# apschera2023uzk/MWR_fast_forward_operators_and_LBLs

Hardware: AMD Instinct MI355X
Metric: TB evaluations/sec (profile x channel x angle) (higher is better)
Workload: dtype f64

## Files before the change

### mwr_fast_forward_operators_and_lbls_amd/csrc/mwrt_absorption.hip.h

```cpp
#pragma once
#include "mwrt_math.hip.h"

namespace mwrt {

typedef const __attribute__((address_space(4))) LineMasks* cmasks;
__device__ __forceinline__ LineMasks load_masks(const LineMasks* table, int chunk) {
  const cmasks q = (cmasks)table + chunk;
  LineMasks lm;
  lm.o2_far = q->o2_far; lm.h2o_far = q->h2o_far; lm.h2o_none = q->h2o_none; lm.h2o_res = q->h2o_res; lm.h2o_sd = q->h2o_sd;
  lm.h2o_sdfar = q->h2o_sdfar; lm.h2o_sdint = q->h2o_sdint;
  lm.h2o_vfar = q->h2o_vfar; lm.o2_vfar = q->o2_vfar; lm.vf_u0 = q->vf_u0; lm.vf_h = q->vf_h; lm.vf_invh = q->vf_invh;
  return lm;
}

struct LevelState {
  double t;
  double p;
  double rho;
  double pdry;
};

__device__ __forceinline__ double goff_gratch_e(double tk, double rh) {
  const double LN10 = 2.302585092994045684;
  const double INV_LN10 = 0.434294481903251828;
  double y = 373.16 / tk;
  double es = -7.90298 * (y - 1.0) + 5.02808 * (flog(y) * INV_LN10)
            - 1.3816e-07 * (fexp(LN10 * (11.344 * (1.0 - (1.0 / y)))) - 1.0)
            + 0.0081328 * (fexp(LN10 * (-3.49149 * (y - 1.0))) - 1.0) + 3.0057148979490314 ;
  return rh * fexp(LN10 * es);
}

__device__ __forceinline__ LevelState level_state(double p_hpa, double tk, double e) {
  const double rvap = (0.01 * 8.314510) / 18.01528;
  double v = 300.0 / tk;
  double ekpa = e / 10.0;
  double pdrykpa = p_hpa / 10.0 - ekpa;
  LevelState s;
  s.t = 300.0 / v;
  s.p = (pdrykpa + ekpa) * 10.0;
  s.rho = ekpa * 10.0 / (rvap * s.t);
  s.pdry = pdrykpa * 10.0;
  return s;
}

struct H2OLine {
  double c1;
  double w0, wsq;
  double sw;
  double sbase;
  double s;
  double base;
};

__device__ __forceinline__ H2OLine h2o_line(cmodel M, int k, double pda, double pvap, double ti, double tiln,
                                            double ti2, bool shifted) {
  H2OLine q;
  const auto& R = M->h2or[k];
  const double fl = R.fl;
  q.w0 = R.w0 * pda * fexp(R.x * tiln) + R.w0s * pvap * fexp(R.xs * tiln);
  double shift = 0.0;
  if (shifted) {
    const double xh = R.xh, xhs = R.xhs, aa = R.aair, as = R.aself;
    double sf = R.sh * pda, ss = R.shs * pvap;
    if (aa != 0.0) sf *= (1.0 - aa * tiln);
    if (as != 0.0) ss *= (1.0 - as * tiln);
    if (xh != 0.0) sf *= fexp(xh * tiln);
    if (xhs != 0.0) ss *= fexp(xhs * tiln);
    shift = sf + ss;
  }
  q.wsq = q.w0 * q.w0;
  q.s = R.s1 * ti2 * fexp(R.b2 * (1.0 - ti));
  q.base = fdiv1(q.w0, 562500.0 + q.wsq);
  q.c1 = fl + shift;
  q.sw = q.s * q.w0;
  q.sbase = q.s * q.base;
  return q;
}

struct FarLine { double P, Q, A2, Bc; };

template <int NFC>
__device__ __forceinline__ void far_quad_accumulate(const double* sfq, const FarLine& a, const FarLine& b,
                                                    const FarLine& c, const FarLine& d, double (&sum)[NFC]) {
  static_assert(NFC % 2 == 0, "frequencies are taken in pairs");
  auto front = [&](const double (&f2s)[2], double (&den)[2], double (&num)[2]) {
#pragma unroll
    for (int g = 0; g < 2; ++g) {
      const double f2 = f2s[g];
      const double d0 = __builtin_fma(f2, f2 + a.A2, a.Bc);
      const double d1 = __builtin_fma(f2, f2 + b.A2, b.Bc);
      const double d2 = __builtin_fma(f2, f2 + c.A2, c.Bc);
      const double d3 = __builtin_fma(f2, f2 + d.A2, d.Bc);
      const double n0 = __builtin_fma(f2, a.P, a.Q);
      const double n1 = __builtin_fma(f2, b.P, b.Q);
      const double n2 = __builtin_fma(f2, c.P, c.Q);
      const double n3 = __builtin_fma(f2, d.P, d.Q);
      const double p01 = d0 * d1, p23 = d2 * d3;
      const double m01 = __builtin_fma(n0, d1, n1 * d0);
      const double m23 = __builtin_fma(n2, d3, n3 * d2);
      den[g] = p01 * p23;
      num[g] = __builtin_fma(m01, p23, m23 * p01);
    }
  };
  double den[2], num[2], r[2];
  double f2c[2] = {sfq[1], sfq[3]};
  double f2n[2] = {sfq[(NFC > 2) ? 5 : 1], sfq[(NFC > 2) ? 7 : 3]};
  front(f2c, den, num);
  r[0] = __builtin_amdgcn_rcp(den[0]); r[1] = __builtin_amdgcn_rcp(den[1]);
#pragma unroll
  for (int j = 0; j < NFC; j += 2) {
    double den_n[2] = {1.0, 1.0}, num_n[2] = {0.0, 0.0}, f2p[2] = {0.0, 0.0};
    if (j + 4 < NFC) { f2p[0] = sfq[2 * (j + 4) + 1]; f2p[1] = sfq[2 * (j + 5) + 1]; }
    MWRT_STAGE();
    if (j + 2 < NFC) front(f2n, den_n, num_n);
    MWRT_STAGE();
    const double e0 = __builtin_fma(-den[0], r[0], 1.0), e1 = __builtin_fma(-den[1], r[1], 1.0);
    r[0] = __builtin_fma(r[0], e0, r[0]); r[1] = __builtin_fma(r[1], e1, r[1]);
    sum[j] = __builtin_fma(num[0], r[0], sum[j]); sum[j + 1] = __builtin_fma(num[1], r[1], sum[j + 1]);
    if (j + 2 < NFC) {
      den[0] = den_n[0]; den[1] = den_n[1]; num[0] = num_n[0]; num[1] = num_n[1];
      r[0] = __builtin_amdgcn_rcp(den[0]); r[1] = __builtin_amdgcn_rcp(den[1]);
      f2n[0] = f2p[0]; f2n[1] = f2p[1];
    }
  }
  MWRT_STAGE();
}

constexpr int VF_TERMS = 8;
__device__ __forceinline__ void vfar_add(const FarLine& fl, double u0, double h, double (&acc)[VF_TERMS]) {
  const double d0 = __builtin_fma(u0, u0 + fl.A2, fl.Bc);
  const double d1h = __builtin_fma(fl.A2, h, (2.0 * u0) * h);
  double rd = __builtin_amdgcn_rcp(d0);
  rd = __builtin_fma(rd, __builtin_fma(-d0, rd, 1.0), rd);
  const double a = -d1h * rd, b = (-(h * h)) * rd;
  double cm2 = __builtin_fma(fl.P, u0, fl.Q) * rd;
  double cm1 = __builtin_fma(a, cm2, (fl.P * h) * rd);
  acc[0] += cm2;
  acc[1] += cm1;
#pragma unroll
  for (int j = 2; j < VF_TERMS; ++j) {
    const double cj = __builtin_fma(a, cm1, b * cm2);
    acc[j] += cj;
    cm2 = cm1; cm1 = cj;
  }
}
template <int NFC>
__device__ __forceinline__ void vfar_eval(const double* sfq, double invh, double mu , const double (&acc)[VF_TERMS], double (&sum)[NFC]) {
  constexpr int G = (NFC % 7 == 0) ? 7 : ((NFC % 4 == 0) ? 4 : 2);
  static_assert(NFC % G == 0, "group width");
#pragma unroll
  for (int j0 = 0; j0 < NFC; j0 += G) {
    double x[G], p[G];
#pragma unroll
    for (int g = 0; g < G; ++g) { x[g] = __builtin_fma(sfq[2 * (j0 + g) + 1], invh, mu); p[g] = acc[VF_TERMS - 1]; }
#pragma unroll
    for (int k = VF_TERMS - 2; k >= 0; --k) {
#pragma unroll
      for (int g = 0; g < G; ++g) p[g] = __builtin_fma(p[g], x[g], acc[k]);
      MWRT_STAGE();
    }
#pragma unroll
    for (int g = 0; g < G; ++g) sum[j0 + g] += p[g];
  }
}

template <int NFC>
__device__ __forceinline__ void far_pair_accumulate(const double* sfq, const FarLine& a, const FarLine& b, double (&sum)[NFC]) {
#pragma unroll
  for (int j = 0; j < NFC; ++j) {
    const double f2 = sfq[2 * j + 1];
    const double d0 = __builtin_fma(f2, f2 + a.A2, a.Bc);
    const double d1 = __builtin_fma(f2, f2 + b.A2, b.Bc);
    const double n0 = __builtin_fma(f2, a.P, a.Q);
    const double n1 = __builtin_fma(f2, b.P, b.Q);
    const double den = d0 * d1;
    const double num = __builtin_fma(n0, d1, n1 * d0);
    double r = __builtin_amdgcn_rcp(den);
    r = __builtin_fma(r, __builtin_fma(-den, r, 1.0), r);
    sum[j] = __builtin_fma(num, r, sum[j]);
  }
}

__device__ __forceinline__ unsigned long long lowest_bits(unsigned long long m, int n) {
  unsigned long long out = 0;
  for (int i = 0; i < n; ++i) { const unsigned long long b = m & (0ull - m); out |= b; m ^= b; }
  return out;
}


template <int NFC, bool NODES = false>
__device__ __forceinline__ void h2o_absorb(cmodel M, const LevelState& L, const double* sfq ,
                                           const LineMasks& lm, double (&awet)[NFC], unsigned excl = 0u,
                                           const double* init_sum = nullptr, double init_bsum = 0.0,
                                           unsigned* failed = nullptr, double* bsum_out = nullptr,
                                           cdoubles sdw = nullptr ) {
  const double t = L.t;
  const double pvap = fdiv(L.rho * t, M->h2o_pvap_div);
  const double pda = L.p - pvap;
  const double den = M->h2o_den_coef * L.rho;
  const double lnc = flog(fdiv(M->h2o_reftcon, t));
  const double con0 = (M->h2o_cf * pda * fexp(M->h2o_xcf * lnc) + M->h2o_cs * pvap * fexp(M->h2o_xcs * lnc)) * pvap;
  const double ti = fdiv(M->h2o_reftline, t);
  const double tiln = flog(ti);
  const double ti2 = fexp(2.5 * tiln);
  const bool shifted = M->h2o_shift_mode != 0;
  double sum[NFC];
#pragma unroll
  for (int j = 0; j < NFC; ++j) sum[j] = init_sum ? init_sum[j] : 0.0;

  const int nl = M->n_h2o;
  const unsigned all = ((nl >= 32) ? 0xffffffffu : ((1u << nl) - 1u)) & ~excl;
  const double fmin = sfq[2 * NFC], fmax = sfq[2 * NFC + 1];
  double bsum = init_bsum;
  const unsigned sd_eff = lm.h2o_sd & ~lm.h2o_sdfar;
  unsigned sd_extra = 0u;
  unsigned deferred = (~lm.h2o_far | lm.h2o_res) & ~sd_eff & ~lm.h2o_none & all;
  const unsigned setA = (MWRT_ABLATE & 2) ? 0u : (lm.h2o_far & ~lm.h2o_res & ~sd_eff & ~lm.h2o_none & all);
  const unsigned setV = NODES ? 0u : (setA & lm.h2o_vfar);
  const unsigned setQ = setA & ~setV;
  const unsigned leftA = (unsigned)lowest_bits(setQ, __builtin_popcount(setQ) & 3);
  const unsigned leftP = (__builtin_popcount(leftA) >= 2) ? (unsigned)lowest_bits(leftA, 2) : 0u;
  deferred |= leftA & ~leftP;
  auto far_setup = [&](int k, FarLine& fl) {
    const H2OLine q = h2o_line(M, k, pda, pvap, ti, tiln, ti2, shifted);
    const bool plain = wave_all_of(q.c1 - fmin < 750.0, fmax - q.c1 < 750.0, q.c1 - fmin > -750.0, fmax + q.c1 < 750.0, fmin + q.c1 > -750.0);
    const double cc = __builtin_fma(q.c1, q.c1, q.wsq);
    fl.A2 = 2.0 * __builtin_fma(-q.c1, q.c1, q.wsq);
    fl.Bc = cc * cc;
    double P = 2.0 * q.sw, bs = 2.0 * q.sbase;
    const bool sdline = M->h2o_w2[k] > 0.0;
    const bool reach = sdline && !wave_all(10.0 * q.w0 < ::fmin(fabs(q.c1 - fmin), fabs(q.c1 - fmax)));
    if (reach || !plain) {
      if constexpr (NODES) *failed |= 1u << k;
      else if (reach) sd_extra |= 1u << k;
      else deferred |= 1u << k;
      P = 0.0; bs = 0.0;
    }
    fl.P = P;
    fl.Q = P * cc;
    bsum += bs;
  };
  if (setV) {
    double acc[VF_TERMS];
#pragma unroll
    for (int j = 0; j < VF_TERMS; ++j) acc[j] = 0.0;
    for (unsigned m = setV; m; m &= m - 1u) {
      FarLine q;
      far_setup(__builtin_ctz(m), q);
      vfar_add(q, lm.vf_u0, lm.vf_h, acc);
    }
    LDS_RELOAD_FENCE();
    vfar_eval<NFC>(sfq, lm.vf_invh, -lm.vf_u0 * lm.vf_invh, acc, sum);
  }
  for (unsigned m = setQ & ~leftA; m;) {
    FarLine q0, q1, q2, q3;
    far_setup(__builtin_ctz(m), q0); m &= m - 1u;
    far_setup(__builtin_ctz(m), q1); m &= m - 1u;
    far_setup(__builtin_ctz(m), q2); m &= m - 1u;
    far_setup(__builtin_ctz(m), q3); m &= m - 1u;
    LDS_RELOAD_FENCE();
    far_quad_accumulate<NFC>(sfq, q0, q1, q2, q3, sum);
  }
  if (leftP) {
    FarLine q0, q1;
    unsigned m = leftP;
    far_setup(__builtin_ctz(m), q0); m &= m - 1u;
    far_setup(__builtin_ctz(m), q1);
    LDS_RELOAD_FENCE();
    far_pair_accumulate<NFC>(sfq, q0, q1, sum);
  }
  if (MWRT_ABLATE & 2) deferred = 0u;
  for (unsigned m = deferred; m; m &= m - 1u) {
    const int k = __builtin_ctz(m);
    const H2OLine q = h2o_line(M, k, pda, pvap, ti, tiln, ti2, shifted);
    const bool d1_in = (q.c1 - fmin < 750.0) && (fmax - q.c1 < 750.0) && (q.c1 - fmin > -750.0);
    const bool d1_out = (q.c1 - fmax >= 750.0) || (fmin - q.c1 >= 750.0);
    const bool d2_in = fmax + q.c1 < 750.0 && fmin + q.c1 > -750.0;
    const bool d2_out = fmin + q.c1 >= 750.0;
    if (wave_all(d1_out && d2_out)) continue;
    if (M->h2o_w2[k] > 0.0 && !wave_all(10.0 * q.w0 < ::fmin(fabs(q.c1 - fmin), fabs(q.c1 - fmax)))) {
      if constexpr (NODES) *failed |= 1u << k; else sd_extra |= 1u << k;
      continue;
    }
    LDS_RELOAD_FENCE();
    if (wave_all(d1_in && d2_in)) {
      bsum = __builtin_fma(2.0, q.sbase, bsum);
#pragma unroll
      for (int j = 0; j < NFC; ++j) {
        const double f = sfq[2 * j];
        const double d1 = f - q.c1;
        const double d2 = f + q.c1;
        const double D1 = __builtin_fma(d1, d1, q.wsq);
        const double D2 = __builtin_fma(d2, d2, q.wsq);
        const double den12 = D1 * D2;
        double r = __builtin_amdgcn_rcp(den12);
        r = __builtin_fma(r, __builtin_fma(-den12, r, 1.0), r);
        sum[j] = __builtin_fma((D1 + D2) * r, q.sw, sum[j]);
      }
    } else if (wave_all(d1_in && d2_out)) {
      bsum += q.sbase;
#pragma unroll
      for (int j = 0; j < NFC; ++j) {
        const double d1 = sfq[2 * j] - q.c1;
        const double D1 = __builtin_fma(d1, d1, q.wsq);
        double r = __builtin_amdgcn_rcp(D1);
        r = __builtin_fma(r, __builtin_fma(-D1, r, 1.0), r);
        sum[j] = __builtin_fma(r, q.sw, sum[j]);
      }
    } else if constexpr (NODES) {
      *failed |= 1u << k;
    } else {
#pragma unroll
      for (int j = 0; j < NFC; ++j) {
        const double f = sfq[2 * j];
        const double d1 = f - q.c1;
        const double d2 = f + q.c1;
        const double D1 = __builtin_fma(d1, d1, q.wsq);
        const double D2 = __builtin_fma(d2, d2, q.wsq);
        const double m1 = (fabs(d1) < 750.0) ? 1.0 : 0.0;
        const double m2 = (fabs(d2) < 750.0) ? 1.0 : 0.0;
        const double num = __builtin_fma(m2, D1, m1 * D2);
        const double r = fdiv1(num, D1 * D2);
        sum[j] = __builtin_fma(r, q.sw, sum[j]);
        sum[j] = __builtin_fma(-(m1 + m2), q.sbase, sum[j]);
      }
    }
  }
  if constexpr (NODES) {
#pragma unroll
    for (int j = 0; j < NFC; ++j) awet[j] = sum[j];
    *bsum_out = bsum;
    return;
  }
#pragma unroll
  for (int j = 0; j < NFC; ++j) sum[j] -= bsum;
  const unsigned setC = (MWRT_ABLATE & 4) ? 0u : ((sd_eff | sd_extra) & all);
  for (unsigned m = setC; m; m &= m - 1u) {
// ... 27 lines not shown
        sum[j] -= inner ? q.sbase : sbase2;
      }
    } else {
#pragma unroll
      for (int j = 0; j < NFC; ++j) {
        const double f = sfq[2 * j];
        const double d1 = f - q.c1;
        const double d2 = f + q.c1;
        const double D1 = __builtin_fma(d1, d1, q.wsq);
        const double D2 = __builtin_fma(d2, d2, q.wsq);
        const double a1 = fabs(d1);
        const double m1 = (a1 < 750.0 && !(a1 < sdlim)) ? 1.0 : 0.0;
        const double m2 = (fabs(d2) < 750.0) ? 1.0 : 0.0;
        const double num = __builtin_fma(m2, D1, m1 * D2);
        const double r = fdiv1(num, D1 * D2);
        sum[j] = __builtin_fma(r, q.sw, sum[j]);
        sum[j] = __builtin_fma(-(m1 + m2), q.sbase, sum[j]);
      }
    }
    LDS_RELOAD_FENCE();
    auto sd_shape = [&](double d1) -> double {
      const cplx xc = cmul(cplx{xre, d1 + xim0}, iden2);
      const cplx xrt = csqrt_principal(xc);
      const cplx w = dcerror_upper(-xrt.im, xrt.re);
      const cplx pxw = cmul(cplx{1.77245385090551603 * xrt.re, 1.77245385090551603 * xrt.im}, w);
      return __builtin_fma(2.0 * (1.0 - pxw.re), iden2.re, 2.0 * pxw.im * iden2.im);
    };
    bool done = false;
    if constexpr (NFC == 16 && !NODES) {
      if (half) {
        done = true;
        const double dmin = ::fmin(fabs(sfq[0] - q.c1), fabs(sfq[2 * 15] - q.c1));
        if (wave_any(dmin < sdlim)) {
          double dn[SD_NODES];
#pragma unroll
          for (int n = 0; n < SD_NODES; ++n) {
            const int j = sd_node_slot(n);
            const double d1 = sfq[2 * j] - q.c1;
            const double sdre = sd_shape(d1);
            const double lres = fdiv1(q.w0, __builtin_fma(d1, d1, q.wsq));
            dn[n] = sdre - lres;
            const double r1 = (fabs(d1) < sdlim) ? sdre - q.base : 0.0;
            sum[j] = __builtin_fma(q.s, r1, sum[j]);
          }
#pragma unroll
          for (int i = 0; i < SD_TARGETS; ++i) {
            const int j = 2 * i + 1;
            double dl = 0.0;
#pragma unroll
            for (int n = 0; n < SD_NODES; ++n) dl = __builtin_fma(sdw[i * SD_NODES + n], dn[n], dl);
            const bool inner = fabs(sfq[2 * j] - q.c1) < sdlim;
            sum[j] = __builtin_fma(q.s, inner ? dl : 0.0, sum[j]);
          }
        }
      }
    }
    if (!done) {
#pragma unroll
      for (int j = 0; j < NFC; ++j) {
        const double d1 = sfq[2 * j] - q.c1;
        const bool inner = fabs(d1) < sdlim;
        if (wave_any(inner)) {
          const double r1 = inner ? sd_shape(d1) - q.base : 0.0;
          sum[j] = __builtin_fma(q.s, r1, sum[j]);
        }
      }
    }
  }
  const bool dry = !(L.rho > 0.0);
#pragma unroll
  for (int j = 0; j < NFC; ++j) {
    const double f2 = sfq[2 * j + 1];
    awet[j] = dry ? 0.0 : (3.183e-05 * den * sum[j] + con0) * f2;
  }
}

struct O2Line {
  double c1, df2;
  double P, Q;
  double cc;
  double dnu;
};

template <int NFC, bool NODES = false>
__device__ __forceinline__ void dry_absorb(cmodel M, const LevelState& L, const double* sfq ,
                                           const LineMasks& lm, double (&adry)[NFC], unsigned long long excl = 0ull,
                                           const double* init_sum = nullptr, unsigned long long* failed = nullptr) {
  const double temp = L.t;
  const double pres = L.p;
  const double th = fdiv(300.0, temp);
  const double th1 = th - 1.0;
  const double lnth = flog(th);
  const double b = fexp(M->o2_x * lnth);
  const double preswv = fdiv(L.rho * temp, M->o2_pvap_div);
  const double presda = pres - preswv;
  const double den = 0.001 * (presda * b + M->o2_wv_factor * preswv * th);
  const double dens = 0.001 * (presda + M->o2_wv_factor * preswv) * th;
  const double dfnr = M->o2_wb300 * den;
  const double pe2 = den * den;
  const bool second = M->o2_mix_mode != 0;
  const double ymul = second ? den : 0.001 * pres * b;
  const bool line1_dens = !second && M->o2_line1_dens;

  double sum[NFC];
#pragma unroll
  for (int j = 0; j < NFC; ++j) sum[j] = init_sum ? init_sum[j] : 0.0;

  long long be_prev = -1;
  double ebe = 1.0;
  auto line_setup = [&](int k) -> O2Line {
    const auto& R = M->o2r[k];
    const double y = ymul * __builtin_fma(R.y1, th1, R.y0);
    double dnu = 0.0, gfac = 1.0;
    if (second) {
      dnu = pe2 * __builtin_fma(R.dnu1, th1, R.dnu0);
      gfac = __builtin_fma(pe2, __builtin_fma(R.g1, th1, R.g0), 1.0);
    }
    const double df = R.w300 * ((k == 0 && line1_dens) ? dens : den);
    const long long be_bits = __builtin_bit_cast(long long, R.be);
    if (be_bits != be_prev) { ebe = fexp(-R.be * th1); be_prev = be_bits; }
    const double str = R.s300rf2 * ebe;
    O2Line q;
    q.dnu = dnu;
    q.c1 = R.f + dnu;
    q.df2 = df * df;
    const double a = (str * df) * gfac;
    const double cb = q.c1 * (str * y);
    q.cc = __builtin_fma(q.c1, q.c1, q.df2);
    q.P = a + cb;
    q.Q = q.cc * (a - cb);
    return q;
  };

  const int nl = M->n_o2;
  const unsigned long long all = ((nl >= 64) ? ~0ull : ((1ull << nl) - 1ull)) & ~excl;
  unsigned long long near = ~lm.o2_far & all;
  const unsigned long long setA = (MWRT_ABLATE & 1) ? 0ull : (lm.o2_far & all);
  const unsigned long long setV = NODES ? 0ull : (setA & lm.o2_vfar);
  const unsigned long long setQ = setA & ~setV;
  const unsigned long long leftA = lowest_bits(setQ, __builtin_popcountll(setQ) & 3);
  const unsigned long long leftP = (__builtin_popcountll(leftA) >= 2) ? lowest_bits(leftA, 2) : 0ull;
  near |= leftA & ~leftP;
  auto far_setup = [&](int k, FarLine& fl) {
    const O2Line q = line_setup(k);
    double P = q.P, Q = q.Q;
    if (!NODES && second && !wave_all(fabs(q.dnu) < FAR_SHIFT_GHZ)) { near |= 1ull << k; P = 0.0; Q = 0.0; }
    fl.P = P; fl.Q = Q;
    fl.A2 = 2.0 * __builtin_fma(-q.c1, q.c1, q.df2);
    fl.Bc = q.cc * q.cc;
  };
  if (setV) {
    double acc[VF_TERMS];
#pragma unroll
    for (int j = 0; j < VF_TERMS; ++j) acc[j] = 0.0;
    for (unsigned long long m = setV; m; m &= m - 1ull) {
      FarLine q;
      far_setup(__builtin_ctzll(m), q);
      vfar_add(q, lm.vf_u0, lm.vf_h, acc);
    }
    LDS_RELOAD_FENCE();
    vfar_eval<NFC>(sfq, lm.vf_invh, -lm.vf_u0 * lm.vf_invh, acc, sum);
  }
  for (unsigned long long m = setQ & ~leftA; m;) {
    FarLine q0, q1, q2, q3;
    far_setup(__builtin_ctzll(m), q0); m &= m - 1ull;
    far_setup(__builtin_ctzll(m), q1); m &= m - 1ull;
    far_setup(__builtin_ctzll(m), q2); m &= m - 1ull;
    far_setup(__builtin_ctzll(m), q3); m &= m - 1ull;
    LDS_RELOAD_FENCE();
    far_quad_accumulate<NFC>(sfq, q0, q1, q2, q3, sum);
  }
  if (leftP) {
    FarLine q0, q1;
    unsigned long long m = leftP;
    far_setup(__builtin_ctzll(m), q0); m &= m - 1ull;
    far_setup(__builtin_ctzll(m), q1);
    LDS_RELOAD_FENCE();
    far_pair_accumulate<NFC>(sfq, q0, q1, sum);
  }
  if (MWRT_ABLATE & 1) near = 0ull;
  be_prev = -1;
  for (unsigned long long m = near; m; m &= m - 1ull) {
    const int k = __builtin_ctzll(m);
    const O2Line q = line_setup(k);
    LDS_RELOAD_FENCE();
#pragma unroll
    for (int j = 0; j < NFC; ++j) {
      const double f = sfq[2 * j], f2 = sfq[2 * j + 1];
      const double d1 = f - q.c1;
      const double d2 = f + q.c1;
      const double D1 = __builtin_fma(d1, d1, q.df2);
      const double D2 = __builtin_fma(d2, d2, q.df2);
      const double den12 = D1 * D2;
      double r = __builtin_amdgcn_rcp(den12);
      r = __builtin_fma(r, __builtin_fma(-den12, r, 1.0), r);
      sum[j] = __builtin_fma(__builtin_fma(f2, q.P, q.Q), r, sum[j]);
    }
  }
  if constexpr (NODES) {
#pragma unroll
    for (int j = 0; j < NFC; ++j) adry[j] = sum[j];
    (void)failed;
    return;
  }
  const double scale2 = 2.0 * M->o2_coef * presda * th * th * th;
  const double pn2 = M->n2_ptot ? pres : L.pdry;
  const double n2c = M->n2_n * M->n2_l * pn2 * pn2 * fexp(M->n2_m * lnth);
  const double nr0 = 0.5 * M->o2_nonres * dfnr;
  const double dfnr2 = dfnr * dfnr;
#pragma unroll
  for (int j = 0; j < NFC; ++j) {
    const double f2 = sfq[2 * j + 1];
    const double hnonres = fdiv(nr0 * f2, th * (f2 + dfnr2));
    double o2 = scale2 * __builtin_fma(sum[j], f2, hnonres);
    o2 = fmax(o2, 0.0);
    adry[j] = o2 + n2c * sfq[2 * NFC + 2 + j] * f2;
  }
}

__device__ __forceinline__ cplx clog_(cplx w) {
  return {0.5 * flog(__builtin_fma(w.re, w.re, w.im * w.im)), atan2(w.im, w.re)};
}

struct CloudLevel {
  int mode;
  double eps0;
  double a, b, c;
  cplx z1, icnorm;
};
constexpr double CLOUD_KICE = 8.18645 * 0.000959553 * (0.1 * 2.302585092994045684) / 29.9792458;

__device__ __forceinline__ CloudLevel cloud_level(cmodel M, double tk) {
  CloudLevel c{};
  c.mode = M->liq_mode;
  if (c.mode == 0) {
    const double theta1 = 1.0 - fdiv(300.0, tk);
    c.eps0 = 77.66 - 103.3 * theta1;
    c.a = 0.0671 * c.eps0;
    const double fp = (316.0 * theta1 + 146.4) * theta1 + 20.2;
    c.b = fdiv(1.0, fp);
    c.c = fdiv(1.0, 39.8 * fp);
  } else {
    const double tc = tk - 273.15;
    const double lth = flog(fdiv(300.0, tk));
    c.eps0 = -43.7527 * fexp(0.05 * lth) + 299.504 * fexp(1.47 * lth) - 399.364 * fexp(2.11 * lth) + 221.327 * fexp(2.31 * lth);
    c.a = 80.69715 * fexp(-tc * (1.0 / 226.45));
    c.b = 1164.023 * fexp(fdiv(-651.4728, tc + 133.07));
    c.c = 4.008724 * fexp(-tc * (1.0 / 103.05));
    const double f1 = 10.46012 + tc * (0.1454962 + tc * (0.063267156 + tc * 0.00093786645));
    c.z1 = cplx{-0.75 * f1, f1};
    c.icnorm = crecip(clog_(cdiv(cplx{-4500.0, 2000.0}, c.z1)));
  }
  return c;
}

__device__ __forceinline__ double liquid_abs(const CloudLevel& c, double f, double denl) {
  cplx eps;
  if (c.mode == 0) {
    const double eps2 = 3.52;
    const cplx t1 = cdiv(cplx{c.eps0 - c.a, 0.0}, cplx{1.0, f * c.b});
    const cplx t2 = cdiv(cplx{c.a - eps2, 0.0}, cplx{1.0, f * c.c});
    eps = cplx{t1.re + t2.re + eps2, t1.im + t2.im};
  } else {
    const cplx z2 = {-4500.0, 2000.0};
    const double hdelta = 0.5 * c.c;
    const cplx kap0 = cdiv(cplx{0.0, -c.a * f}, cplx{c.b, f});
    const cplx lp = clog_(cdiv(cplx{-z2.re, f - z2.im}, cplx{-c.z1.re, f - c.z1.im}));
    const cplx lj = clog_(cdiv(cplx{-z2.re, f + z2.im}, cplx{-c.z1.re, f + c.z1.im}));
    const cplx chip = cmul(cplx{hdelta * lp.re, hdelta * lp.im}, c.icnorm);
    const cplx chij = cmul(cplx{hdelta * lj.re, hdelta * lj.im}, cplx{c.icnorm.re, -c.icnorm.im});
    eps = cplx{c.eps0 + (kap0.re + (chip.re + chij.re - c.c)), kap0.im + (chip.im + chij.im)};
  }
  const cplx re = cdiv(cplx{eps.re - 1.0, eps.im}, cplx{eps.re + 2.0, eps.im});
  return -0.06286 * re.im * f * denl;
}

__device__ __forceinline__ double thayer_refindex(double p, double tk, double e) {
  const double pa = p - e, tc = tk - 273.16, tk2 = tk * tk, tc2 = tc * tc;
  const double rza = 1.0 + pa * (5.79e-07 * (1.0 + 0.52 / tk) - (0.00094611 * tc) / tk2);
  const double rzw = 1.0 + 1650.0 * (e / (tk * tk2)) * (1.0 - 0.01317 * tc + 0.000175 * tc2 + 1.44e-06 * (tc2 * tc));
  const double wetn = (64.79 * (e / tk) + 377600.0 * (e / tk2)) * rzw;
  const double dryn = 77.6036 * (pa / tk) * rza;
  return 1.0 + (dryn + wetn) * 1e-06;
}

template <int NFC>
__device__ __forceinline__ void x_absorb(cmodel M, double tk, double p, double numden, const double* sfq, double (&adry)[NFC]) {
  const double ti = fdiv(M->x_reft, tk);
  const double tiln = flog(ti);
  const double qvinv = (M->x_qvib_t > 0.0) ? 1.0 - fexp(-fdiv(M->x_qvib_t, tk)) : 1.0;
  const double sq = 4.3e-07 * fsqrt(fdiv(tk, M->x_mass));
  double sum[NFC];
#pragma unroll
  for (int j = 0; j < NFC; ++j) sum[j] = 0.0;
  const int nx = M->n_x;
  for (int k = 0; k < nx; ++k) {
    const double fl = M->x_fl[k];
    const double wc = M->x_w[k] * p * fexp(M->x_x[k] * tiln);
    const double bd = sq * fl;
    const double w = 0.5346 * wc + fsqrt(__builtin_fma(0.2166 * wc, wc, 0.6931 * (bd * bd)));
    const double wsq = w * w;
    const double sw = (M->x_s1[k] * fexp(M->x_b[k] * (1.0 - ti))) * fdiv(w, fl * fl);
    LDS_RELOAD_FENCE();
#pragma unroll
    for (int j = 0; j < NFC; ++j) {
      const double f = sfq[2 * j];
      const double d1 = f - fl, d2 = f + fl;
      const double D1 = __builtin_fma(d1, d1, wsq), D2 = __builtin_fma(d2, d2, wsq);
      const double den12 = D1 * D2;
      double r = __builtin_amdgcn_rcp(den12);
      r = __builtin_fma(r, __builtin_fma(-den12, r, 1.0), r);
      sum[j] = __builtin_fma((D1 + D2) * r, sw, sum[j]);
    }
  }
  const double pref = ((M->x_coef * numden) * qvinv) * fexp(2.5 * tiln);
#pragma unroll
  for (int j = 0; j < NFC; ++j) adry[j] = __builtin_fma(pref * sfq[2 * j + 1], sum[j], adry[j]);
}

}
```

### mwr_fast_forward_operators_and_lbls_amd/csrc/mwrt_fused.hip.h

```cpp
#pragma once
#include "mwrt_absorption.hip.h"
#include "mwrt_layer.hip.h"

namespace mwrt {

__device__ __forceinline__ void blank_outputs(const FusedArgs& A, int64_t prof, int jbase, int nfc, int tid, int nthreads) {
  const double qnan = __builtin_nan("");
  const int nang = A.nang, nlev = A.nlev;
  for (int it = tid; it < nfc * nang; it += nthreads) {
    const int j = it / nang, a = it % nang;
    const int64_t o = (prof * nang + a) * A.nf + jbase + j;
    A.tb[o] = qnan;
    if (A.tbatm) A.tbatm[o] = qnan;
    if (A.tmr) A.tmr[o] = qnan;
    if (A.tauwet) A.tauwet[o] = qnan;
    if (A.taudry) A.taudry[o] = qnan;
    if (A.tauliq) A.tauliq[o] = qnan;
    if (A.tauice) A.tauice[o] = qnan;
  }
  if (A.taulay) for (int it = tid; it < nfc * nlev; it += nthreads)
    A.taulay[(prof * A.nf + jbase + it / nlev) * nlev + it % nlev] = qnan;
}

typedef const __attribute__((address_space(3))) double* ldoubles;
template <class Step>
__device__ __forceinline__ void rte_segment(const double* tau_seg, const double* bof_seg, int seglen, Step step) {
  ldoubles tp = (ldoubles)tau_seg, bp = (ldoubles)bof_seg;
  asm volatile("" : "+v"(tp), "+v"(bp));
  double t0 = tp[0], t1 = tp[1], b0 = bp[0], b1 = bp[1];
  for (int n = seglen >> 2; n > 0; --n) {
    const double t2 = tp[2], t3 = tp[3];
    step(t0, b0);
    const double b2 = bp[2], b3 = bp[3];
    step(t1, b1);
    t0 = tp[4]; t1 = tp[5];
    step(t2, b2);
    b0 = bp[4]; b1 = bp[5];
    step(t3, b3);
    tp += 4; bp += 4;
  }
  const int rest = seglen & 3;
  if (rest > 0) step(t0, b0);
  if (rest > 1) step(t1, b1);
  if (rest > 2) step(tp[2], bp[2]);
}

template <int NFC, int NFK, int MAXT, bool OPT = false, bool EXTRAS = false, bool ALPHA = false>
__global__ void __launch_bounds__(MAXT, (MAXT <= 256 ? (EXTRAS ? MWRT_MIN_WAVES : (ALPHA ? 4 : 3)) : 1))
k_tb_fused(const FusedArgs A) {
  constexpr int NPASS = (NFC + NFK - 1) / NFK;
  static_assert(NPASS <= 2, "LaunchGeom carries the split of two passes");
  extern __shared__ __attribute__((aligned(16))) double lds[];
  const int tid = threadIdx.x;
  const int lane = tid & (WAVE - 1);
  const int wave = tid / WAVE;
  const int nthreads = blockDim.x;
  const int nwaves = nthreads / WAVE;
  const int64_t prof = blockIdx.x;
  const int mi = (int)(prof / A.nprof_in);
  const int64_t pin = prof - mi * A.nprof_in;
  const int jbase = blockIdx.y * NFC;
  const int nfc = min(NFC, A.nf - jbase);
  const int nlev = A.nlev, nang = A.nang, ld = A.g.ldrow;
  const cmodel M = (cmodel)A.Ms[mi];
  const cdoubles cfrq = (cdoubles)A.frq;
  const cdoubles cam = (cdoubles)A.airmass;

  double* tau = lds;
  double* bof = tau + (size_t)NFK * ld;
  double* part = bof + (size_t)NFK * ld;
  double* scratch = part + (size_t)A.g.npart;
  double* edge = scratch + 16;
  constexpr int GRP = 16;
  const int ngrp = nthreads / GRP;
  float* gmax = (float*)(edge + (size_t)nwaves * 2 * NFC);
  int* wcnt = (int*)(gmax + (size_t)NFK * ngrp);
  int* perm = wcnt + nwaves;
  __shared__ int s_flag;
  __shared__ double sfq[5 * NFC + 2];

  MWRT_STAMP(0);
#if MWRT_PHASE_CLOCK
  if (A.phase && lane == 0) {
    A.phase[((int64_t)blockIdx.x * 4 + wave) * 10 + 8] = (long long)__builtin_amdgcn_s_getreg((31 << 11) | 4);
    A.phase[((int64_t)blockIdx.x * 4 + wave) * 10 + 9] = (long long)__builtin_amdgcn_s_getreg((31 << 11) | 20);
  }
#endif
  if (tid == 0) s_flag = 0;
  if (tid < NFC) {
    const double f = cfrq[jbase + min(tid, nfc - 1)];
    sfq[2 * tid] = f; sfq[2 * tid + 1] = f * f;
    double fdep = 1.0;
    if (M->n2_fdep) { const double q = f * (1.0 / 450.0); fdep = 0.5 + fdiv(0.5, 1.0 + q * q); }
    sfq[2 * NFC + 2 + tid] = fdep;
    sfq[3 * NFC + 2 + tid] = fdiv(1.0, f);
    sfq[4 * NFC + 2 + tid] = fdiv(1.0, fexp(fdiv(f * (1e9 * M->planck_h / M->boltzmann_k), M->t_cosmic)) - 1.0);
  }
  if (tid == WAVE - 1) {
    double lo = cfrq[jbase], hi = lo;
    for (int j = 1; j < nfc; ++j) { const double f = cfrq[jbase + j]; lo = fmin(lo, f); hi = fmax(hi, f); }
    sfq[2 * NFC] = lo; sfq[2 * NFC + 1] = hi;
  }
  __syncthreads();

  const bool active = tid < nlev;
  const bool wave_live = wave * WAVE < nlev;
  const int64_t off = pin * nlev + (active ? tid : 0);
  const double zi = A.z[off], ti = A.t[off];
  const double pi = ALPHA ? 0.0 : A.p[off], rhi = ALPHA ? 0.0 : A.rh[off];
  if (active && (isnan(zi) || isnan(pi) || isnan(ti) || isnan(rhi))) atomicOr(&s_flag, 1);
  double awet[NFC], adry[NFC];
  if constexpr (ALPHA) {
    bool bad = false;
    if (wave_live) {
#pragma unroll
      for (int j = 0; j < NFC; ++j) {
        const int64_t o = (pin * A.nf + jbase + min(j, nfc - 1)) * nlev + (active ? tid : 0);
        awet[j] = A.awet_in[o];
        adry[j] = A.adry_in[o];
        bad = bad || isnan(awet[j]) || isnan(adry[j]);
      }
    } else {
#pragma unroll
      for (int j = 0; j < NFC; ++j) { awet[j] = 0.0; adry[j] = 0.0; }
    }
    if (active && bad) atomicOr(&s_flag, 1);
  }
  double denl = 0.0, deni = 0.0, o3n = 0.0;
  if constexpr (OPT) {
    if (A.denliq) denl = A.denliq[off];
    if (A.denice) deni = A.denice[off];
    if (A.o3n) o3n = A.o3n[off];
    if (active && (isnan(denl) || isnan(deni) || isnan(o3n))) atomicOr(&s_flag, 1);
  }
  __syncthreads();
  if (s_flag) {
    blank_outputs(A, prof, jbase, nfc, tid, nthreads);
    if (tid == 0) A.valid[prof] = 0;
    return;
  }

  if constexpr (!ALPHA) {
    const double e = goff_gratch_e(ti, rhi);
    const LevelState L = level_state(pi, ti, e);
    const LineMasks lm = load_masks(A.masks[mi], blockIdx.y);
    MWRT_STAMP(1);
    MWRT_SETPRIO(3);
    h2o_absorb<NFC>(M, L, sfq, lm, awet);
    MWRT_STAMP(2);
    MWRT_SETPRIO(2);
    dry_absorb<NFC>(M, L, sfq, lm, adry);
    MWRT_SETPRIO(1);
    MWRT_STAMP(3);
    if constexpr (OPT) {
      if (A.o3n) x_absorb<NFC>(M, ti, pi, o3n, sfq, adry);
    }
  }
  if (lane == WAVE - 1) {
#pragma unroll
    for (int j = 0; j < NFC; ++j) { edge[wave * 2 * NFC + j] = awet[j]; edge[wave * 2 * NFC + NFC + j] = adry[j]; }
  }
  __syncthreads();
  double tw[EXTRAS ? NFC : 1], td[NFC];
  bool neg = false;
  {
    const double z0 = A.z[pin * nlev];
    const double dz = (active && tid > 0) ? ((zi - z0) - (A.z[off - 1] - z0)) : 0.0;
    const bool seam = (lane == 0) && (wave > 0);
    const bool has_prev = active && tid > 0;
    if (!wave_live) {
#pragma unroll
      for (int j = 0; j < NFC; ++j) { td[j] = 0.0; if constexpr (EXTRAS) tw[j] = 0.0; }
    } else
#pragma unroll
    for (int j = 0; j < NFC; ++j) {
#pragma clang fp contract(off)
      double pw = __shfl_up(awet[j], 1, WAVE);
      double pd = __shfl_up(adry[j], 1, WAVE);
      if (seam) { pw = edge[(wave - 1) * 2 * NFC + j]; pd = edge[(wave - 1) * 2 * NFC + NFC + j]; }
      const double lw = layer_value(awet[j], pw, neg, has_prev), ld_ = layer_value(adry[j], pd, neg, has_prev);
      const double twj = has_prev ? lw * dz : 0.0;
      const double tdj = has_prev ? ld_ * dz : 0.0;
      if constexpr (EXTRAS) { tw[j] = twj; td[j] = tdj; }
      else td[j] = twj + tdj;
    }
  }
  constexpr bool CLOUD_ROWS = OPT && EXTRAS;
  double tl[CLOUD_ROWS ? NFC : 1], tci[CLOUD_ROWS ? NFC : 1];
  if constexpr (OPT) {
#pragma unroll
    for (int j = 0; j < (CLOUD_ROWS ? NFC : 1); ++j) { tl[j] = 0.0; tci[j] = 0.0; }
    const bool cloud_here = active && (denl > 0.0 || deni > 0.0);
    if ((A.denliq || A.denice) && __syncthreads_or(cloud_here)) {
      auto row = [&](int j) -> double* { return (j < NFK ? tau + (size_t)j * ld : bof + (size_t)(j - NFK) * ld); };
      {
        const CloudLevel cl = cloud_level(M, ti);
        if (active) {
#pragma unroll
          for (int j = 0; j < NFC; ++j) row(j)[tid] = (denl > 0.0) ? liquid_abs(cl, sfq[2 * j], denl) : 0.0;
        }
      }
      __syncthreads();
      const bool has_below = active && tid > 0;
      const double deni_prev = (has_below && A.denice) ? A.denice[off - 1] : 0.0;
      const double z0 = A.z[pin * nlev];
      const double dz = has_below ? ((zi - z0) - (A.z[off - 1] - z0)) : 0.0;
#pragma unroll
      for (int j = 0; j < NFC; ++j) {
        const double f = sfq[2 * j];
        const double al = active ? row(j)[tid] : 0.0;
        const double pl = has_below ? row(j)[tid - 1] : 0.0;
        const double ai = (deni > 0.0) ? CLOUD_KICE * f * deni : 0.0;
        const double pc = (deni_prev > 0.0) ? CLOUD_KICE * f * deni_prev : 0.0;
        const double ll = layer_value<false>(al, pl, neg, has_below), li = layer_value<false>(ai, pc, neg, has_below);
        const double tlj = has_below ? ll * dz : 0.0;
        const double tij = has_below ? li * dz : 0.0;
        if constexpr (CLOUD_ROWS) { tl[j] = tlj; tci[j] = tij; }
        else td[j] = (td[j] + tij) + tlj;
      }
      __syncthreads();
    }
  }
  MWRT_STAMP(4);
  if (neg) atomicOr(&s_flag, 2);
  __syncthreads();
  if (s_flag) {
    blank_outputs(A, prof, jbase, nfc, tid, nthreads);
    if (tid == 0) A.valid[prof] = 2;
    return;
  }
  const double hk = 1e9 * M->planck_h / M->boltzmann_k;
  const double inv_hk = 1e-9 * M->boltzmann_k / M->planck_h;
  bool want_tau = false;
  if constexpr (EXTRAS) {
    if (A.taulay && active) {
#pragma unroll
      for (int j = 0; j < NFC; ++j)
        if (j < nfc) {
          double tz = tw[j] + td[j];
          if constexpr (CLOUD_ROWS) tz = (tz + tci[j]) + tl[j];
          A.taulay[(prof * A.nf + jbase + j) * nlev + tid] = tz;
        }
    }
    want_tau = (A.tauwet != nullptr) || (A.taudry != nullptr) || (A.tauliq != nullptr) || (A.tauice != nullptr);
  }

  for (int k = nlev + tid; k < ld; k += nthreads) {
#pragma unroll
    for (int jj = 0; jj < NFK; ++jj) { tau[jj * ld + k] = 0.0; bof[jj * ld + k] = 0.0; }
  }

#pragma unroll
  for (int h = 0; h < NPASS; ++h) {
    const int nfk = min(NFK, nfc - h * NFK);
    if (nfk <= 0) break;
    if (h > 0) MWRT_SETPRIO(0);
    if (h > 0) __syncthreads();
    const int nseg = A.g.nseg[h], seglen = A.g.seglen[h];
    const int npairs = nfk * nang;
    const int items = (MWRT_ABLATE & 8) ? 0 : npairs * nseg;
    const bool sorted = !(OPT && A.amf) && items <= nthreads && seglen >= K2_SORT_MIN_SEGLEN;
    if (wave_live) {
      const double hkt = fdiv(hk, ti);
      const double kth = ti * inv_hk;
#pragma unroll
      for (int jj = 0; jj < NFK; ++jj) {
        const int j = h * NFK + jj;
        if (j < NFC) {
          double tz = td[j];
          if constexpr (EXTRAS) tz = tw[j] + td[j];
          if constexpr (CLOUD_ROWS) tz = (tz + tci[j]) + tl[j];
          const double bz = planck_b(sfq[2 * j] * hkt, sfq[3 * NFC + 2 + j] * kth);
          if (active) { tau[jj * ld + tid] = tz; bof[jj * ld + tid] = bz; }
          if (sorted) {
            const float m = row16_max(active ? (float)tz * 1.0000005f : 0.0f);
            if ((lane & (GRP - 1)) == 0) gmax[jj * ngrp + tid / GRP] = m;
          }
// ... 198 lines not shown
```

### mwr_fast_forward_operators_and_lbls_amd/csrc/mwrt_plan.h

```cpp
#pragma once
#include <stddef.h>
#include <stdint.h>
#include <vector>
#include "../../include/mwrt.h"

namespace mwrt {

constexpr int WAVE = 64;

struct LaunchGeom {
  int nseg[2];
  int seglen[2];
  int npart;
  int ldrow;
  unsigned magic_nseg[2];
  unsigned magic_nang;
};

constexpr double FAR_MIN_GHZ = 0.2;
constexpr double FAR_SHIFT_GHZ = 0.05;
constexpr double FAR_H2O_GHZ = 5.0;

struct LineMasks {
  unsigned long long o2_far;
  unsigned h2o_far;
  unsigned h2o_none;
  unsigned h2o_res;
  unsigned h2o_sd;
  unsigned h2o_sdfar;
  unsigned h2o_sdint;
  unsigned h2o_vfar;
  unsigned long long o2_vfar;
  double vf_u0, vf_h, vf_invh;
};

constexpr double VF_RATIO_MAX = 0.016;
constexpr int VF_MIN_FREQS = 7;
constexpr int VF_MIN_LINES = 4;

constexpr int SD_NODES = 9, SD_TARGETS = 7;
constexpr int sd_node_slot(int n) { return n < 8 ? 2 * n : 15; }

constexpr int MAX_MULTI = 8;

constexpr int NFK = 8;
constexpr int K2_SORT_MIN_SEGLEN = 16;

constexpr int TAU_NFC = 16;
constexpr int tau_threads(int nlev) { return ((nlev - 1 + (WAVE - 2)) / (WAVE - 1)) * WAVE; }
constexpr int lanes_for(int nlev) { return ((nlev + WAVE - 1) / WAVE) * WAVE; }

constexpr int WIN_NODES = 16;
constexpr int WIN_NODES_H = 8;
constexpr int WIN_CHUNKS = 8;
constexpr int WIN_CHUNKS_MAX = 16;
constexpr int WIN_NFC = 16;

struct WinDesc {
  double fnode[WIN_NODES];
  double fnode_h[WIN_NODES_H];
  double flo, fhi;
  unsigned long long o2_far;
  unsigned h2o_far_both, h2o_far_res;
  int first_chunk, nchunks;
  int pad0, pad1;
};

constexpr int RTE_THREADS = 256;

constexpr double WIN_MARGIN_GHZ = 4.0;
constexpr double WIN_H2O_MARGIN_GHZ = 30.0;
constexpr double WIN_MAX_SPAN_GHZ = 6.0;
constexpr double WIN_CUTOFF_GUARD_GHZ = 5.0;

unsigned magic_of(int d);

bool plan_fused(int lds_max, int nfc, int nlev, int nf, int nang, LaunchGeom* g, size_t* lds, int threads = 0);
int pick_nfc(int nf);
int pick_nfc_fused(int chunk_width, int lds_max, int nlev, int nf, int nang);

bool any_nan(const double* x, int n);
bool all_nan(const double* x, int n);
bool airmass_of(const double* elev, int nang, std::vector<double>* am);
int rte_tau_angles(int rem);
int tau_pitch_of(int nf);

size_t absorb_win_lds_bytes(int threads);
bool windows_eligible(const double* frq, int nf);
enum class AbsorbRoute { every_line, windowed, refused  };
AbsorbRoute absorption_route(int mode, int lds_max, const double* frq, int nf, int threads);

void chunk_masks(const mwrt_model_desc& t, const double* frq, int nf, int nfc, std::vector<LineMasks>* out);

struct WindowSet {
  std::vector<WinDesc> wins;
  std::vector<double> lag, lag_h;
  std::vector<double> lag_sd;
};
void build_windows(const mwrt_model_desc& t, const double* frq, int nf, WindowSet* ws);

struct WindowLayout { size_t off_lag, off_lagh, off_lagsd, total; };
WindowLayout window_layout(int nwin, int nf);
void pack_windows(const WindowSet& ws, int nf, std::vector<char>* blob);

struct RowArray { double* p; size_t per; };
void blank_rows(const uint8_t* valid, int64_t nrows, const RowArray* arrays, int narrays);

}
```

Before: 1.006 billion.

## Group far-line quads into shared fractions and park wet absorption in LDS

Far-wing line contributions are now folded into one running numerator/denominator per frequency across up to five quads, so a single reciprocal closes each group instead of one per quad. For kernels with at most 512 threads, wet absorption is written to the LDS tau rows after the H2O pass and read back for the layer integration. This frees registers, and inputs like z, t, p and ozone are reloaded rather than kept live. The grouping trades reciprocals for more multiplies and a larger product denominator, which risks overflow or precision loss. The LDS parking adds shared-memory traffic.

```diff
diff --git a/mwr_fast_forward_operators_and_lbls_amd/csrc/mwrt_absorption.hip.h b/mwr_fast_forward_operators_and_lbls_amd/csrc/mwrt_absorption.hip.h
--- a/mwr_fast_forward_operators_and_lbls_amd/csrc/mwrt_absorption.hip.h
+++ b/mwr_fast_forward_operators_and_lbls_amd/csrc/mwrt_absorption.hip.h
@@ -79,28 +79,29 @@
 
 struct FarLine { double P, Q, A2, Bc; };
 
+__device__ __forceinline__ void far_quad_terms(double f2, const FarLine& a, const FarLine& b, const FarLine& c, const FarLine& d,
+                                               double& den, double& num) {
+  const double d0 = __builtin_fma(f2, f2 + a.A2, a.Bc);
+  const double d1 = __builtin_fma(f2, f2 + b.A2, b.Bc);
+  const double d2 = __builtin_fma(f2, f2 + c.A2, c.Bc);
+  const double d3 = __builtin_fma(f2, f2 + d.A2, d.Bc);
+  const double n0 = __builtin_fma(f2, a.P, a.Q);
+  const double n1 = __builtin_fma(f2, b.P, b.Q);
+  const double n2 = __builtin_fma(f2, c.P, c.Q);
+  const double n3 = __builtin_fma(f2, d.P, d.Q);
+  const double p01 = d0 * d1, p23 = d2 * d3;
+  const double m01 = __builtin_fma(n0, d1, n1 * d0);
+  const double m23 = __builtin_fma(n2, d3, n3 * d2);
+  den = p01 * p23;
+  num = __builtin_fma(m01, p23, m23 * p01);
+}
 template <int NFC>
 __device__ __forceinline__ void far_quad_accumulate(const double* sfq, const FarLine& a, const FarLine& b,
                                                     const FarLine& c, const FarLine& d, double (&sum)[NFC]) {
   static_assert(NFC % 2 == 0, "frequencies are taken in pairs");
   auto front = [&](const double (&f2s)[2], double (&den)[2], double (&num)[2]) {
 #pragma unroll
-    for (int g = 0; g < 2; ++g) {
-      const double f2 = f2s[g];
-      const double d0 = __builtin_fma(f2, f2 + a.A2, a.Bc);
-      const double d1 = __builtin_fma(f2, f2 + b.A2, b.Bc);
-      const double d2 = __builtin_fma(f2, f2 + c.A2, c.Bc);
-      const double d3 = __builtin_fma(f2, f2 + d.A2, d.Bc);
-      const double n0 = __builtin_fma(f2, a.P, a.Q);
-      const double n1 = __builtin_fma(f2, b.P, b.Q);
-      const double n2 = __builtin_fma(f2, c.P, c.Q);
-      const double n3 = __builtin_fma(f2, d.P, d.Q);
-      const double p01 = d0 * d1, p23 = d2 * d3;
-      const double m01 = __builtin_fma(n0, d1, n1 * d0);
-      const double m23 = __builtin_fma(n2, d3, n3 * d2);
-      den[g] = p01 * p23;
-      num[g] = __builtin_fma(m01, p23, m23 * p01);
-    }
+    for (int g = 0; g < 2; ++g) far_quad_terms(f2s[g], a, b, c, d, den[g], num[g]);
   };
   double den[2], num[2], r[2];
   double f2c[2] = {sfq[1], sfq[3]};
@@ -126,6 +127,56 @@
   MWRT_STAGE();
 }
 
+constexpr int FAR_GROUP_QUADS = 5;
+template <int NFC, bool FIRST>
+__device__ __forceinline__ void far_quad_fraction(const double* sfq, const FarLine& a, const FarLine& b, const FarLine& c,
+                                                  const FarLine& d, const double (&sum)[NFC], double (&N)[NFC], double (&D)[NFC]) {
+#pragma unroll
+  for (int j = 0; j < NFC; ++j) {
+    double den, num;
+    far_quad_terms(sfq[2 * j + 1], a, b, c, d, den, num);
+    if constexpr (FIRST) {
+      N[j] = __builtin_fma(sum[j], den, num);
+      D[j] = den;
+    } else {
+      N[j] = __builtin_fma(N[j], den, num * D[j]);
+      D[j] *= den;
+    }
+  }
+}
+template <int NFC>
+__device__ __forceinline__ void far_group_close(const double (&N)[NFC], const double (&D)[NFC], double (&sum)[NFC]) {
+  double r[NFC];
+#pragma unroll
+  for (int j = 0; j < NFC; ++j) r[j] = __builtin_amdgcn_rcp(D[j]);
+#pragma unroll
+  for (int j = 0; j < NFC; ++j) r[j] = __builtin_fma(r[j], __builtin_fma(-D[j], r[j], 1.0), r[j]);
+#pragma unroll
+  for (int j = 0; j < NFC; ++j) sum[j] = N[j] * r[j];
+}
+template <int NFC, class Mask, class Setup>
+__device__ __forceinline__ void far_groups_accumulate(const double* sfq, Mask m, Setup&& setup, double (&sum)[NFC]) {
+  auto next_quad = [&](FarLine (&q)[4]) {
+#pragma unroll
+    for (int i = 0; i < 4; ++i) { setup(__builtin_ctzll((unsigned long long)m), q[i]); m &= m - Mask(1); }
+    LDS_RELOAD_FENCE();
+  };
+  while (m) {
+    double N[NFC], D[NFC];
+    {
+      FarLine q[4];
+      next_quad(q);
+      far_quad_fraction<NFC, true>(sfq, q[0], q[1], q[2], q[3], sum, N, D);
+    }
+    for (int g = 1; g < FAR_GROUP_QUADS && m; ++g) {
+      FarLine q[4];
+      next_quad(q);
+      far_quad_fraction<NFC, false>(sfq, q[0], q[1], q[2], q[3], sum, N, D);
+    }
+    far_group_close<NFC>(N, D, sum);
+  }
+}
+
 constexpr int VF_TERMS = 8;
 __device__ __forceinline__ void vfar_add(const FarLine& fl, double u0, double h, double (&acc)[VF_TERMS]) {
   const double d0 = __builtin_fma(u0, u0 + fl.A2, fl.Bc);
@@ -188,7 +239,7 @@
 }
 
 
-template <int NFC, bool NODES = false>
+template <int NFC, bool NODES = false, bool GROUPED = false>
 __device__ __forceinline__ void h2o_absorb(cmodel M, const LevelState& L, const double* sfq ,
                                            const LineMasks& lm, double (&awet)[NFC], unsigned excl = 0u,
                                            const double* init_sum = nullptr, double init_bsum = 0.0,
@@ -209,15 +260,15 @@
   for (int j = 0; j < NFC; ++j) sum[j] = init_sum ? init_sum[j] : 0.0;
 
   const int nl = M->n_h2o;
-  const unsigned all = ((nl >= 32) ? 0xffffffffu : ((1u << nl) - 1u)) & ~excl;
+  const unsigned all = h2o_lines_all(nl) & ~excl;
   const double fmin = sfq[2 * NFC], fmax = sfq[2 * NFC + 1];
   double bsum = init_bsum;
-  const unsigned sd_eff = lm.h2o_sd & ~lm.h2o_sdfar;
+  const unsigned sd_eff = h2o_sd_near(lm);
   unsigned sd_extra = 0u;
   unsigned deferred = (~lm.h2o_far | lm.h2o_res) & ~sd_eff & ~lm.h2o_none & all;
-  const unsigned setA = (MWRT_ABLATE & 2) ? 0u : (lm.h2o_far & ~lm.h2o_res & ~sd_eff & ~lm.h2o_none & all);
-  const unsigned setV = NODES ? 0u : (setA & lm.h2o_vfar);
-  const unsigned setQ = setA & ~setV;
+  const unsigned setA = (MWRT_ABLATE & 2) ? 0u : h2o_far_set(lm, all);
+  const unsigned setV = h2o_vfar_set(lm, setA, NODES);
+  const unsigned setQ = h2o_quad_set(lm, setA, NODES);
   const unsigned leftA = (unsigned)lowest_bits(setQ, __builtin_popcount(setQ) & 3);
   const unsigned leftP = (__builtin_popcount(leftA) >= 2) ? (unsigned)lowest_bits(leftA, 2) : 0u;
   deferred |= leftA & ~leftP;
@@ -252,7 +303,8 @@
     LDS_RELOAD_FENCE();
     vfar_eval<NFC>(sfq, lm.vf_invh, -lm.vf_u0 * lm.vf_invh, acc, sum);
   }
-  for (unsigned m = setQ & ~leftA; m;) {
+  if constexpr (GROUPED) far_groups_accumulate<NFC>(sfq, setQ & ~leftA, far_setup, sum);
+  else for (unsigned m = setQ & ~leftA; m;) {
     FarLine q0, q1, q2, q3;
     far_setup(__builtin_ctz(m), q0); m &= m - 1u;
     far_setup(__builtin_ctz(m), q1); m &= m - 1u;
@@ -446,7 +498,7 @@
   double dnu;
 };
 
-template <int NFC, bool NODES = false>
+template <int NFC, bool NODES = false, bool GROUPED = false>
 __device__ __forceinline__ void dry_absorb(cmodel M, const LevelState& L, const double* sfq ,
                                            const LineMasks& lm, double (&adry)[NFC], unsigned long long excl = 0ull,
                                            const double* init_sum = nullptr, unsigned long long* failed = nullptr) {
@@ -497,11 +549,11 @@
   };
 
   const int nl = M->n_o2;
-  const unsigned long long all = ((nl >= 64) ? ~0ull : ((1ull << nl) - 1ull)) & ~excl;
+  const unsigned long long all = o2_lines_all(nl) & ~excl;
   unsigned long long near = ~lm.o2_far & all;
-  const unsigned long long setA = (MWRT_ABLATE & 1) ? 0ull : (lm.o2_far & all);
-  const unsigned long long setV = NODES ? 0ull : (setA & lm.o2_vfar);
-  const unsigned long long setQ = setA & ~setV;
+  const unsigned long long setA = (MWRT_ABLATE & 1) ? 0ull : o2_far_set(lm, all);
+  const unsigned long long setV = o2_vfar_set(lm, setA, NODES);
+  const unsigned long long setQ = o2_quad_set(lm, setA, NODES);
   const unsigned long long leftA = lowest_bits(setQ, __builtin_popcountll(setQ) & 3);
   const unsigned long long leftP = (__builtin_popcountll(leftA) >= 2) ? lowest_bits(leftA, 2) : 0ull;
   near |= leftA & ~leftP;
@@ -525,7 +577,8 @@
     LDS_RELOAD_FENCE();
     vfar_eval<NFC>(sfq, lm.vf_invh, -lm.vf_u0 * lm.vf_invh, acc, sum);
   }
-  for (unsigned long long m = setQ & ~leftA; m;) {
+  if constexpr (GROUPED) far_groups_accumulate<NFC>(sfq, setQ & ~leftA, far_setup, sum);
+  else for (unsigned long long m = setQ & ~leftA; m;) {
     FarLine q0, q1, q2, q3;
     far_setup(__builtin_ctzll(m), q0); m &= m - 1ull;
     far_setup(__builtin_ctzll(m), q1); m &= m - 1ull;
@@ -595,27 +648,28 @@
 constexpr double CLOUD_KICE = 8.18645 * 0.000959553 * (0.1 * 2.302585092994045684) / 29.9792458;
 
 __device__ __forceinline__ CloudLevel cloud_level(cmodel M, double tk) {
-  CloudLevel c{};
-  c.mode = M->liq_mode;
-  if (c.mode == 0) {
+  const int mode = M->liq_mode;
+  double eps0, a, b, c3;
+  cplx z1 = {0.0, 0.0}, icnorm = {0.0, 0.0};
+  if (mode == 0) {
     const double theta1 = 1.0 - fdiv(300.0, tk);
-    c.eps0 = 77.66 - 103.3 * theta1;
-    c.a = 0.0671 * c.eps0;
+    eps0 = 77.66 - 103.3 * theta1;
+    a = 0.0671 * eps0;
     const double fp = (316.0 * theta1 + 146.4) * theta1 + 20.2;
-    c.b = fdiv(1.0, fp);
-    c.c = fdiv(1.0, 39.8 * fp);
+    b = fdiv(1.0, fp);
+    c3 = fdiv(1.0, 39.8 * fp);
   } else {
     const double tc = tk - 273.15;
     const double lth = flog(fdiv(300.0, tk));
-    c.eps0 = -43.7527 * fexp(0.05 * lth) + 299.504 * fexp(1.47 * lth) - 399.364 * fexp(2.11 * lth) + 221.327 * fexp(2.31 * lth);
-    c.a = 80.69715 * fexp(-tc * (1.0 / 226.45));
-    c.b = 1164.023 * fexp(fdiv(-651.4728, tc + 133.07));
-    c.c = 4.008724 * fexp(-tc * (1.0 / 103.05));
+    eps0 = -43.7527 * fexp(0.05 * lth) + 299.504 * fexp(1.47 * lth) - 399.364 * fexp(2.11 * lth) + 221.327 * fexp(2.31 * lth);
+    a = 80.69715 * fexp(-tc * (1.0 / 226.45));
+    b = 1164.023 * fexp(fdiv(-651.4728, tc + 133.07));
+    c3 = 4.008724 * fexp(-tc * (1.0 / 103.05));
     const double f1 = 10.46012 + tc * (0.1454962 + tc * (0.063267156 + tc * 0.00093786645));
-    c.z1 = cplx{-0.75 * f1, f1};
-    c.icnorm = crecip(clog_(cdiv(cplx{-4500.0, 2000.0}, c.z1)));
-  }
-  return c;
+    z1 = cplx{-0.75 * f1, f1};
+    icnorm = crecip(clog_(cdiv(cplx{-4500.0, 2000.0}, z1)));
+  }
+  return CloudLevel{mode, eps0, a, b, c3, z1, icnorm};
 }
 
 __device__ __forceinline__ double liquid_abs(const CloudLevel& c, double f, double denl) {
diff --git a/mwr_fast_forward_operators_and_lbls_amd/csrc/mwrt_fused.hip.h b/mwr_fast_forward_operators_and_lbls_amd/csrc/mwrt_fused.hip.h
--- a/mwr_fast_forward_operators_and_lbls_amd/csrc/mwrt_fused.hip.h
+++ b/mwr_fast_forward_operators_and_lbls_amd/csrc/mwrt_fused.hip.h
@@ -71,6 +71,9 @@
   double* part = bof + (size_t)NFK * ld;
   double* scratch = part + (size_t)A.g.npart;
   double* edge = scratch + 16;
+  auto row = [&](int j) -> double* { return (j < NFK ? tau + (size_t)j * ld : bof + (size_t)(j - NFK) * ld); };
+  constexpr bool GROUPED = MAXT <= 512;
+  constexpr bool PARK = !ALPHA && GROUPED;
   constexpr int GRP = 16;
   const int ngrp = nthreads / GRP;
   float* gmax = (float*)(edge + (size_t)nwaves * 2 * NFC);
@@ -106,7 +109,7 @@
   const bool active = tid < nlev;
   const bool wave_live = wave * WAVE < nlev;
   const int64_t off = pin * nlev + (active ? tid : 0);
-  const double zi = A.z[off], ti = A.t[off];
+  double zi = A.z[off], ti = A.t[off];
   const double pi = ALPHA ? 0.0 : A.p[off], rhi = ALPHA ? 0.0 : A.rh[off];
   if (active && (isnan(zi) || isnan(pi) || isnan(ti) || isnan(rhi))) atomicOr(&s_flag, 1);
   double awet[NFC], adry[NFC];
@@ -146,21 +149,34 @@
     const LineMasks lm = load_masks(A.masks[mi], blockIdx.y);
     MWRT_STAMP(1);
     MWRT_SETPRIO(3);
-    h2o_absorb<NFC>(M, L, sfq, lm, awet);
+    h2o_absorb<NFC, false, GROUPED>(M, L, sfq, lm, awet);
+    if constexpr (PARK) {
+      if (active) {
+#pragma unroll
+        for (int j = 0; j < NFC; ++j) row(j)[tid] = awet[j];
+      }
+    }
     MWRT_STAMP(2);
     MWRT_SETPRIO(2);
-    dry_absorb<NFC>(M, L, sfq, lm, adry);
+    dry_absorb<NFC, false, GROUPED>(M, L, sfq, lm, adry);
     MWRT_SETPRIO(1);
     MWRT_STAMP(3);
     if constexpr (OPT) {
-      if (A.o3n) x_absorb<NFC>(M, ti, pi, o3n, sfq, adry);
+      if (A.o3n) {
+        LDS_RELOAD_FENCE();
+        x_absorb<NFC>(M, A.t[off], A.p[off], A.o3n[off], sfq, adry);
+      }
     }
   }
   if (lane == WAVE - 1) {
 #pragma unroll
-    for (int j = 0; j < NFC; ++j) { edge[wave * 2 * NFC + j] = awet[j]; edge[wave * 2 * NFC + NFC + j] = adry[j]; }
+    for (int j = 0; j < NFC; ++j) {
+      if constexpr (!PARK) edge[wave * 2 * NFC + j] = awet[j];
+      edge[wave * 2 * NFC + NFC + j] = adry[j];
+    }
   }
   __syncthreads();
+  if constexpr (OPT) { LDS_RELOAD_FENCE(); zi = A.z[off]; ti = A.t[off]; }
   double tw[EXTRAS ? NFC : 1], td[NFC];
   bool neg = false;
   {
@@ -168,6 +184,13 @@
     const double dz = (active && tid > 0) ? ((zi - z0) - (A.z[off - 1] - z0)) : 0.0;
     const bool seam = (lane == 0) && (wave > 0);
     const bool has_prev = active && tid > 0;
+    [[maybe_unused]] ldoubles wrow = nullptr;
+    [[maybe_unused]] double pw_next = 0.0, aw_next = 0.0;
+    if constexpr (PARK) {
+      wrow = (ldoubles)(tau + (has_prev ? tid - 1 : 0));
+      asm volatile("" : "+v"(wrow));
+      if (wave_live) { pw_next = wrow[0]; aw_next = wrow[1]; }
+    }
     if (!wave_live) {
 #pragma unroll
       for (int j = 0; j < NFC; ++j) { td[j] = 0.0; if constexpr (EXTRAS) tw[j] = 0.0; }
@@ -175,10 +198,18 @@
 #pragma unroll
     for (int j = 0; j < NFC; ++j) {
 #pragma clang fp contract(off)
-      double pw = __shfl_up(awet[j], 1, WAVE);
+      double aw, pw;
+      if constexpr (PARK) {
+        aw = aw_next; pw = pw_next;
+        if (j + 1 < NFC) { wrow += ld; pw_next = wrow[0]; aw_next = wrow[1]; }
+      } else {
+        aw = awet[j];
+        pw = __shfl_up(awet[j], 1, WAVE);
+        if (seam) pw = edge[(wave - 1) * 2 * NFC + j];
+      }
       double pd = __shfl_up(adry[j], 1, WAVE);
-      if (seam) { pw = edge[(wave - 1) * 2 * NFC + j]; pd = edge[(wave - 1) * 2 * NFC + NFC + j]; }
-      const double lw = layer_value(awet[j], pw, neg, has_prev), ld_ = layer_value(adry[j], pd, neg, has_prev);
+      if (seam) pd = edge[(wave - 1) * 2 * NFC + NFC + j];
+      const double lw = layer_value(aw, pw, neg, has_prev), ld_ = layer_value(adry[j], pd, neg, has_prev);
       const double twj = has_prev ? lw * dz : 0.0;
       const double tdj = has_prev ? ld_ * dz : 0.0;
       if constexpr (EXTRAS) { tw[j] = twj; td[j] = tdj; }
@@ -192,7 +223,6 @@
     for (int j = 0; j < (CLOUD_ROWS ? NFC : 1); ++j) { tl[j] = 0.0; tci[j] = 0.0; }
     const bool cloud_here = active && (denl > 0.0 || deni > 0.0);
     if ((A.denliq || A.denice) && __syncthreads_or(cloud_here)) {
-      auto row = [&](int j) -> double* { return (j < NFK ? tau + (size_t)j * ld : bof + (size_t)(j - NFK) * ld); };
       {
         const CloudLevel cl = cloud_level(M, ti);
         if (active) {
diff --git a/mwr_fast_forward_operators_and_lbls_amd/csrc/mwrt_plan.h b/mwr_fast_forward_operators_and_lbls_amd/csrc/mwrt_plan.h
--- a/mwr_fast_forward_operators_and_lbls_amd/csrc/mwrt_plan.h
+++ b/mwr_fast_forward_operators_and_lbls_amd/csrc/mwrt_plan.h
@@ -33,6 +33,18 @@
   unsigned long long o2_vfar;
   double vf_u0, vf_h, vf_invh;
 };
+
+constexpr unsigned long long o2_lines_all(int n) { return n >= 64 ? ~0ull : ((1ull << n) - 1ull); }
+constexpr unsigned h2o_lines_all(int n) { return n >= 32 ? 0xffffffffu : ((1u << n) - 1u); }
+constexpr unsigned long long o2_far_set(const LineMasks& lm, unsigned long long all) { return lm.o2_far & all; }
+constexpr unsigned long long o2_vfar_set(const LineMasks& lm, unsigned long long far, bool nodes) { return nodes ? 0ull : (far & lm.o2_vfar); }
+constexpr unsigned long long o2_quad_set(const LineMasks& lm, unsigned long long far, bool nodes) { return far & ~o2_vfar_set(lm, far, nodes); }
+constexpr unsigned h2o_sd_near(const LineMasks& lm) { return lm.h2o_sd & ~lm.h2o_sdfar; }
+constexpr unsigned h2o_far_set(const LineMasks& lm, unsigned all) {
+  return lm.h2o_far & ~lm.h2o_res & ~h2o_sd_near(lm) & ~lm.h2o_none & all;
+}
+constexpr unsigned h2o_vfar_set(const LineMasks& lm, unsigned far, bool nodes) { return nodes ? 0u : (far & lm.h2o_vfar); }
+constexpr unsigned h2o_quad_set(const LineMasks& lm, unsigned far, bool nodes) { return far & ~h2o_vfar_set(lm, far, nodes); }
 
 constexpr double VF_RATIO_MAX = 0.016;
 constexpr int VF_MIN_FREQS = 7;
```

Measured after the change: 1.021 billion, median of 6. 1.01x the previous value.
